# lars-frogner/Impact

Measured on AMD Instinct MI355X. Metric: voxels stepped/sec + remesh tris/sec, 512^3 grid, 1/2/4/8 MI355X, higher is better.
Workload: dtype i8 voxels, f32 SDF/mesh arithmetic, f64 moments; 1 GPU; config-2 SDF asteroid x2.05 -> 502^3 grid = 512^3 stored voxels (32768 chunks); parallelism=single GPU, voxels_per_gpu=134217728, regions=1, triangles=1813104

## Files before the change

### impact_amd/csrc/derive.hip

```cpp
#include "device_common.hpp"
#include "chunk_passes.hpp"
#include "table_roles.hpp"
#include "many.hpp"

#ifndef IVX_POL_SWEEP_PLANES
#define IVX_POL_SWEEP_PLANES IVX_ST_WT
#endif
#ifndef IVX_DERIVE_WAVES
#define IVX_DERIVE_WAVES 6
#endif

namespace {

struct DeriveParams {
    uint32_t cx, cy, cz;
};

__device__ __forceinline__ uint32_t row_mask(uint4 s) {
    uint32_t w[4] = {s.x, s.y, s.z, s.w};
    uint32_t m = 0;
#pragma unroll
    for (int q = 0; q < 4; ++q) m |= ((((w[q] >> 7) & 0x01010101u) * 0x00204081u >> 21) & 0xFu) << (4 * q);
    return m;
}

__device__ __forceinline__ uint32_t nbr_row_mask(const GridView& g, const ivx_chunk_info* info, size_t c, uint32_t off) {
    const uint32_t gen = info[c].gen_kind;
    const uint32_t rm = row_mask(*reinterpret_cast<const uint4*>(g.sdf + c * IVX_CHUNK_VOXELS + off));
    return gen == KIND_NONUNIFORM ? rm : (gen == KIND_UNIFORM ? 0xFFFFu : 0u);
}

struct ChunkPreArgs {
    GridView g;
    ivx_chunk_info* info;
    uint32_t* bbox;
    uint32_t* mesh_counts;
    uint8_t* chunk_class;
    uint8_t* touch;
    uint32_t* rparent;
    uint32_t* work_counts;
    uint32_t* next_work_count;
    uint32_t* active_list;
    ivx_roles::PresetArgs preset;
    uint32_t defer_ghost, pad_;
    unsigned long long* tick;
};
__device__ __forceinline__ void chunk_settle(const GridView& g, const ChunkPreArgs& a, uint32_t chunk, const ivx_chunk_info& own) {
    const uint32_t gen = own.gen_kind;
    const bool solid = gen == KIND_UNIFORM;
    ivx_chunk_info rec = own;
    rec.kind = (uint8_t)gen;
    rec.flags = 0;
    rec.face_dist = solid ? 0x555 : 0;
    rec.uniform_type = solid ? (own.kind == KIND_NONUNIFORM ? g.type[(size_t)chunk * IVX_CHUNK_VOXELS] : own.uniform_type) : (uint8_t)0;
    rec.region_count = solid ? 1 : 0;
    rec.boundary_region_count = solid ? 1 : 0;
    a.info[chunk] = rec;
    a.bbox[chunk] = solid ? (0x80000000u | (15u << 4) | (15u << 12) | (15u << 20)) : 0u;
    a.mesh_counts[2 * chunk] = 0;
    a.mesh_counts[2 * chunk + 1] = 0;
    a.touch[chunk] = solid ? 7 : 0;
    if (solid) a.rparent[(size_t)chunk * 256] = chunk * 256u;
}
__device__ __forceinline__ void chunk_pre_body(const ChunkPreArgs& a, uint32_t bid, uint32_t) {
    const GridView& g = a.g;
    ivx_chunk_info* __restrict__ info = a.info;
    uint32_t* __restrict__ bbox = a.bbox;
    uint32_t* __restrict__ mesh_counts = a.mesh_counts;
    uint8_t* __restrict__ chunk_class = a.chunk_class;
    uint8_t* __restrict__ touch = a.touch;
    uint32_t* __restrict__ rparent = a.rparent;
    uint32_t* __restrict__ work_counts = a.work_counts;
    uint32_t* __restrict__ next_work_count = a.next_work_count;
    uint32_t* __restrict__ active_list = a.active_list;
    __shared__ uint32_t s_w[4];
    __shared__ uint32_t s_base;
    const uint32_t tid = threadIdx.x, lane = tid & 63u, wave = tid >> 6;
    ivx_roles::role_preset(a.preset, bid * 256u + tid);
    if (bid == 0 && tid == 0) next_work_count[0] = 0u;
    const uint32_t n_chunks = g.cx * g.cy * g.cz;
    const uint32_t chunk = bid * 256u + tid;
    const bool live = chunk < n_chunks;
    bool settled = false, pending = false;
    if (live) {
        const ivx_chunk_info own = info[chunk];
        const uint32_t gen = own.gen_kind;
        settled = gen == KIND_VOID;
        if (gen == KIND_UNIFORM) {
            const int ck = chunk % g.cz, cj = (chunk / g.cz) % g.cy, ci = chunk / (g.cz * g.cy);
            if (cj > 0 && ck > 0 && cj + 1 < (int)g.cy && ck + 1 < (int)g.cz) {
                const uint32_t sx = g.cy * g.cz, sy = g.cz;
                const bool ghost_lo = ci == 0 && g.ghost_info[0] != nullptr, ghost_hi = ci + 1 == (int)g.cx && g.ghost_info[1] != nullptr;
                const bool defer = a.defer_ghost != 0u && (ghost_lo || ghost_hi);
                const bool x_lo = ci > 0 ? info[chunk - sx].gen_kind == KIND_UNIFORM : (ghost_lo && (defer || g.ghost_info[0][cj * g.cz + ck].gen_kind == KIND_UNIFORM));
                const bool x_hi =
                    ci + 1 < (int)g.cx ? info[chunk + sx].gen_kind == KIND_UNIFORM : (ghost_hi && (defer || g.ghost_info[1][cj * g.cz + ck].gen_kind == KIND_UNIFORM));
                settled = x_lo && x_hi && info[chunk - sy].gen_kind == KIND_UNIFORM && info[chunk + sy].gen_kind == KIND_UNIFORM &&
                          info[chunk - 1].gen_kind == KIND_UNIFORM && info[chunk + 1].gen_kind == KIND_UNIFORM;
                if (settled && defer) settled = false, pending = true;
            }
        }
        if (settled) chunk_settle(g, a, chunk, own);
        chunk_class[chunk] = pending ? 2 : (settled ? 1 : 0);
    }
    const bool active = live && !settled && !pending;
    const unsigned long long bal = __ballot(active);
    if (lane == 0) s_w[wave] = (uint32_t)__popcll(bal);
    __syncthreads();
    if (tid == 0) s_base = atomicAdd(&work_counts[0], (s_w[0] + s_w[1]) + (s_w[2] + s_w[3]));
    __syncthreads();
    if (active) {
        uint32_t off = s_base + (uint32_t)__popcll(bal & ((1ull << lane) - 1ull));
        for (uint32_t w = 0; w < wave; ++w) off += s_w[w];
        active_list[off] = chunk;
    }
}
__global__ __launch_bounds__(256) void k_chunk_pre(ChunkPreArgs a) {
    ivx_stage_stamp(a.tick);
    chunk_pre_body(a, blockIdx.x, gridDim.x);
}
IVX_MANY_TWIN(k_chunk_pre_many, ChunkPreArgs, chunk_pre_body, __launch_bounds__(256))
IVX_MANY_LAUNCHER(many_chunk_pre, k_chunk_pre_many, ChunkPreArgs, 256)

__global__ __launch_bounds__(256) void k_face_settle(ChunkPreArgs a) {
    const GridView& g = a.g;
    const uint32_t cols = g.cy * g.cz, t = blockIdx.x * 256u + threadIdx.x;
    if (t >= 2u * cols) return;
    const uint32_t side = t / cols, col = t % cols;
    if (side == 1u && g.cx == 1u) return;
    const uint32_t chunk = (side ? g.cx - 1u : 0u) * cols + col;
    if (a.chunk_class[chunk] != 2) return;
    const ivx_chunk_info own = a.info[chunk];
    bool uniform = true;
    if (chunk < cols && g.ghost_info[0]) uniform = uniform && g.ghost_info[0][col].gen_kind == KIND_UNIFORM;
    if (chunk >= (g.cx - 1u) * cols && g.ghost_info[1]) uniform = uniform && g.ghost_info[1][col].gen_kind == KIND_UNIFORM;
    if (uniform) {
        chunk_settle(g, a, chunk, own);
        a.chunk_class[chunk] = 1;
    } else {
        a.chunk_class[chunk] = 0;
        a.active_list[atomicAdd(&a.work_counts[0], 1u)] = chunk;
    }
}

struct DeriveLoads {
    uint2 own_rec;
    uint4 own_sd, own_types, nrow;
// ... 52 lines not shown
    const float* dens;
    double* chunk_moments;
};

struct DeriveBox {
    uint32_t n, derive_blocks;
    uint32_t lo[3], cc[3];
    uint32_t* out_list;
};
__device__ __forceinline__ void role_region_reset(uint32_t bid, const GridView& g, const DeriveBox& box, const ivx_chunk_info* __restrict__ info,
                                                  uint32_t* __restrict__ rparent, uint32_t* __restrict__ rscalar, uint32_t* __restrict__ multi_list) {
    const uint32_t chunk = bid * 256u + threadIdx.x;
    if (chunk >= g.cx * g.cy * g.cz) return;
    const uint32_t ck = chunk % g.cz, cj = (chunk / g.cz) % g.cy, ci = chunk / (g.cz * g.cy);
    if (ci - box.lo[0] < box.cc[0] && cj - box.lo[1] < box.cc[1] && ck - box.lo[2] < box.cc[2]) return;
    const uint32_t rc = info[chunk].region_count;
    for (uint32_t r = 0; r < rc; ++r) rparent[(size_t)chunk * 256 + r] = chunk * 256u + r;
    if (rc > 1u) multi_list[atomicAdd(&rscalar[2], 1u)] = chunk;
}

struct DeriveArgs {
    GridView g;
    int8_t* sdf_rw;
    uint8_t* type_rw;
    uint8_t* flags_out;
    ivx_chunk_info* info;
    uint32_t* bbox;
    uint8_t* touch;
    uint16_t* signs;
    uint8_t* kface_out;
    const uint32_t* work_counts;
    uint32_t* active_list;
    const uint32_t* list_in;
    DeriveFused fz;
    uint32_t signs_type, x_part;
    DeriveBox box;
    unsigned long long* tick;
};
template <bool SIGNS>
__device__ __forceinline__ void derive_body(const DeriveArgs& a_, uint32_t bid_, uint32_t nb_) {
    const GridView& g = a_.g;
    int8_t* __restrict__ sdf_rw = a_.sdf_rw;
    uint8_t* __restrict__ type_rw = a_.type_rw;
    uint8_t* __restrict__ flags_out = a_.flags_out;
    ivx_chunk_info* __restrict__ info = a_.info;
    uint32_t* __restrict__ bbox = a_.bbox;
    uint8_t* __restrict__ touch = a_.touch;
    uint16_t* __restrict__ signs = a_.signs;
    uint8_t* __restrict__ kface_out = a_.kface_out;
    const uint32_t* __restrict__ work_counts = a_.work_counts;
    uint32_t* __restrict__ active_list = a_.active_list;
    const uint32_t* __restrict__ list_in = a_.list_in;
    const DeriveFused& fz = a_.fz;
    const uint32_t signs_type = a_.signs_type;
    const DeriveBox& box = a_.box;
    __shared__ uint32_t occ[18][18];
    __shared__ uint32_t cnt[13];
    __shared__ CclShared s_ccl;
    __shared__ float s_dens[256];
    __shared__ uint16_t s_mtab[256];
    double (*s_red)[10] = reinterpret_cast<double (*)[10]>(s_ccl.par);
    const uint32_t tid = threadIdx.x;
    if (!SIGNS && box.n && bid_ >= box.derive_blocks) {
        role_region_reset(bid_ - box.derive_blocks, g, box, info, fz.rparent, fz.rscalar, fz.multi_list);
        return;
    }
// ... 346 lines not shown
        o[3] = r3;
        o[4] = r2 + r5;
        o[5] = r0 * cx + r5;
        o[6] = r0 * cx + r2;
        o[7] = r1 * qx;
        o[8] = r4;
        o[9] = r3 * qx;
    }
}

__device__ __forceinline__ void derive_wave_body(const DeriveArgs& a_) {
    const GridView& g = a_.g;
    uint8_t* __restrict__ flags_out = a_.flags_out;
    int8_t* __restrict__ sdf_rw = a_.sdf_rw;
    uint8_t* __restrict__ type_rw = a_.type_rw;
    ivx_chunk_info* __restrict__ info = a_.info;
    uint16_t* __restrict__ signs = a_.signs;
    uint8_t* __restrict__ kface_out = a_.kface_out;
    uint32_t* __restrict__ active_list = a_.active_list;
    const uint32_t* __restrict__ list_in = a_.list_in;
    const DeriveFused& fz = a_.fz;
    __shared__ float s_dens[256];
    __shared__ uint16_t s_mtab[256];
    __shared__ uint16_t s_occ[4][18 * 18 + 4];
    __shared__ double s_red_all[4][16][10];
    const uint32_t tid = threadIdx.x, lane = tid & 63u;
    const uint32_t wave = (uint32_t)__builtin_amdgcn_readfirstlane((int)(tid >> 6));
    uint16_t* occ = s_occ[wave];
    double (*s_red)[10] = s_red_all[wave];
    if (fz.parts & IVX_PART_MOMENTS) s_dens[tid] = fz.dens[tid], s_mtab[tid] = moments_table_entry(tid);
    __syncthreads();
    const uint32_t la = lane >> 4, j = lane & 15u;
    const uint32_t n_active = a_.work_counts[0];
    const uint32_t n_walk = gridDim.x * 4u;
    const uint32_t sx = g.cy * g.cz;
    const uint32_t* sw = reinterpret_cast<const uint32_t*>(g.signs);
    for (uint32_t li = ivx_xcd_remap(blockIdx.x, gridDim.x) * 4u + wave; li < n_active; li += n_walk) {
    IVX_TW(g, li, 0);
    const uint32_t chunk = IVX_LIST_CHUNK(list_in[li]);
    const int ck = chunk % g.cz, cj = (chunk / g.cz) % g.cy, ci = chunk / sx;
    const size_t base = (size_t)chunk * IVX_CHUNK_VOXELS;
    const bool has_zlo = ck > 0, has_zhi = ck + 1 < (int)g.cz;
    const size_t c_lo = has_zlo ? (size_t)chunk - 1 : (size_t)chunk, c_hi = has_zhi ? (size_t)chunk + 1 : (size_t)chunk;
    const uint32_t nf = la, nr = j;
    bool n_present;
    size_t nc;
    uint32_t noff;
    if (nf == 0) n_present = ci > 0, nc = (size_t)chunk - sx, noff = 240u + nr;
    else if (nf == 1) n_present = ci + 1 < (int)g.cx, nc = (size_t)chunk + sx, noff = nr;
    else if (nf == 2) n_present = cj > 0, nc = (size_t)chunk - g.cz, noff = nr * 16u + 15u;
    else n_present = cj + 1 < (int)g.cy, nc = (size_t)chunk + g.cz, noff = nr * 16u;
    if (!n_present) nc = chunk;
    uint2 own_rec = reinterpret_cast<const uint2*>(info)[chunk];
    uint32_t gen_lo = reinterpret_cast<const uint32_t*>(info)[2 * c_lo], gen_hi = reinterpret_cast<const uint32_t*>(info)[2 * c_hi];
    uint32_t ngen = reinterpret_cast<const uint32_t*>(info)[2 * nc];
    uint32_t type0 = *reinterpret_cast<const uint32_t*>(g.type + base);
    uint32_t nrow = sw[(nc * 256 + noff) >> 1];
    uint32_t ow[4], bl[4], bh[4];
#pragma unroll
    for (int q = 0; q < 4; ++q) {
        const uint32_t r = (4u * la + q) * 16u + j;
        ow[q] = sw[((size_t)chunk * 256 + r) >> 1];
        bl[q] = sw[(c_lo * 256 + r) >> 1];
        bh[q] = sw[(c_hi * 256 + r) >> 1];
    }
    asm volatile("" : "+v"(own_rec.x), "+v"(own_rec.y), "+v"(gen_lo), "+v"(gen_hi), "+v"(ngen), "+v"(type0), "+v"(nrow));
    asm volatile("" : "+v"(ow[0]), "+v"(ow[1]), "+v"(ow[2]), "+v"(ow[3]), "+v"(bl[0]), "+v"(bl[1]), "+v"(bl[2]), "+v"(bl[3]));
    asm volatile("" : "+v"(bh[0]), "+v"(bh[1]), "+v"(bh[2]), "+v"(bh[3]));
    own_rec.x = (uint32_t)__builtin_amdgcn_readfirstlane((int)own_rec.x), own_rec.y = (uint32_t)__builtin_amdgcn_readfirstlane((int)own_rec.y);
    gen_lo = ((uint32_t)__builtin_amdgcn_readfirstlane((int)gen_lo) >> 8) & 0xFFu, gen_hi = ((uint32_t)__builtin_amdgcn_readfirstlane((int)gen_hi) >> 8) & 0xFFu;
// ... 258 lines not shown
        } else {
            ci_.flags = 0;
            ci_.face_dist = 0;
        }
        info[chunk] = ci_;
    }
    IVX_TW(g, li, 5);
    ivx_wave_lds_sync();
    }
}
__global__ __launch_bounds__(256) __attribute__((amdgpu_waves_per_eu(IVX_DERIVE_WAVE_WAVES, 8))) void k_derive_wave(DeriveArgs a) {
    ivx_stage_stamp(a.tick);
    derive_wave_body(a);
}

struct ListRebuildArgs {
    GridView g;
    const ivx_chunk_info* info;
    uint32_t* work_counts;
    uint32_t* next_work_count;
    uint32_t* active_list;
    uint32_t* mesh_counts;
};
__device__ __forceinline__ void list_rebuild_body(const ListRebuildArgs& a, uint32_t bid, uint32_t) {
    const GridView& g = a.g;
    const ivx_chunk_info* __restrict__ info = a.info;
    uint32_t* __restrict__ work_counts = a.work_counts;
    uint32_t* __restrict__ next_work_count = a.next_work_count;
    uint32_t* __restrict__ active_list = a.active_list;
    uint32_t* __restrict__ mesh_counts = a.mesh_counts;
    __shared__ uint32_t s_w[4];
    __shared__ uint32_t s_base;
    const uint32_t tid = threadIdx.x, lane = tid & 63u, wave = tid >> 6;
    if (bid == 0 && tid == 0) next_work_count[0] = 0u;
    const uint32_t n_chunks = g.cx * g.cy * g.cz;
    const uint32_t chunk = bid * 256u + tid;
    const bool live = chunk < n_chunks;
    bool settled = false;
    uint32_t entry = 0;
    if (live) {
        const ivx_chunk_info own = info[chunk];
        const uint32_t gen = own.gen_kind;
        settled = gen == KIND_VOID;
        if (gen == KIND_UNIFORM) {
            const int ck = chunk % g.cz, cj = (chunk / g.cz) % g.cy, ci = chunk / (g.cz * g.cy);
            if (cj > 0 && ck > 0 && cj + 1 < (int)g.cy && ck + 1 < (int)g.cz) {
                const uint32_t sx = g.cy * g.cz, sy = g.cz;
                const bool x_lo = ci > 0 ? info[chunk - sx].gen_kind == KIND_UNIFORM
                                         : (g.ghost_info[0] != nullptr && g.ghost_info[0][cj * g.cz + ck].gen_kind == KIND_UNIFORM);
                const bool x_hi = ci + 1 < (int)g.cx ? info[chunk + sx].gen_kind == KIND_UNIFORM
                                                     : (g.ghost_info[1] != nullptr && g.ghost_info[1][cj * g.cz + ck].gen_kind == KIND_UNIFORM);
                settled = x_lo && x_hi && info[chunk - sy].gen_kind == KIND_UNIFORM && info[chunk + sy].gen_kind == KIND_UNIFORM &&
                          info[chunk - 1].gen_kind == KIND_UNIFORM && info[chunk + 1].gen_kind == KIND_UNIFORM;
            }
        }
        const uint32_t kind = own.kind;
        const bool exposed = kind == KIND_NONUNIFORM && (own.flags & CF_FULLY_OBSCURED) != CF_FULLY_OBSCURED;
        entry = chunk | (kind << 24) | (gen << 26) | (exposed ? (1u << 28) : 0u);
        if (settled) {
            mesh_counts[2 * chunk] = 0;
            mesh_counts[2 * chunk + 1] = 0;
        }
    }
    const bool active = live && !settled;
    const unsigned long long bal = __ballot(active);
    if (lane == 0) s_w[wave] = (uint32_t)__popcll(bal);
    __syncthreads();
// ... 47 lines not shown
                if (q < 6) atomicMin(&red[q], v[q]);
                else atomicMax(&red[q], v[q]);
            }
        }
        __syncthreads();
        if (tid < 6) atomicMin(&raw[tid], red[tid]);
        else if (tid < 12) atomicMax(&raw[tid], red[tid]);
    }
}

__global__ __launch_bounds__(256) void k_step_preset(ivx_roles::PresetArgs preset) { ivx_roles::role_preset(preset, blockIdx.x * 256u + threadIdx.x); }

__global__ __launch_bounds__(256) void k_materialize(uint32_t n_chunks, const ivx_chunk_info* __restrict__ info, int8_t* __restrict__ sdf,
                                                     uint8_t* __restrict__ type, uint8_t* __restrict__ flags, uint8_t* __restrict__ labels) {
    const uint32_t chunk = ivx_xcd_remap(blockIdx.x, n_chunks);
    const ivx_chunk_info ci = info[chunk];
    if (ci.kind == KIND_NONUNIFORM) return;
    const size_t o = (size_t)chunk * IVX_CHUNK_VOXELS + (size_t)threadIdx.x * 16;
    const uint32_t s = ivx_uniform_sdf(ci.kind) * 0x01010101u, t = ivx_uniform_type(ci) * 0x01010101u;
    const uint32_t f = ivx_uniform_flags(ci.kind) * 0x01010101u, l = ivx_uniform_label(ci.kind) * 0x01010101u;
    *reinterpret_cast<uint4*>(sdf + o) = make_uint4(s, s, s, s);
    *reinterpret_cast<uint4*>(type + o) = make_uint4(t, t, t, t);
    *reinterpret_cast<uint4*>(flags + o) = make_uint4(f, f, f, f);
    *reinterpret_cast<uint4*>(labels + o) = make_uint4(l, l, l, l);
}

static DeriveArgs derive_args(ivx_grid* g, const GridView& v, const DeriveFused& fz) {
    DeriveArgs da;
    memset(&da, 0, sizeof(da));
    da.g = v, da.sdf_rw = g->sdf, da.type_rw = g->type, da.flags_out = g->flags, da.info = g->info, da.bbox = g->chunk_bbox, da.touch = g->chunk_touch;
    da.signs = g->chunk_signs, da.kface_out = g->kface, da.work_counts = ivx_wc(g), da.active_list = g->active_list, da.list_in = g->active_list, da.fz = fz;
    return da;
}
static_assert(sizeof(DeriveArgs) % 8 == 0 && sizeof(ChunkPreArgs) % 8 == 0 && sizeof(ListRebuildArgs) % 8 == 0, "argument blocks travel as 8-byte words");
static const int s_many_registered_derive =
    (ivx_many_register(IVX_MK_DERIVE_PLANES, many_derive_planes, sizeof(DeriveArgs)), ivx_many_register(IVX_MK_DERIVE_SIGNS, many_derive_signs, sizeof(DeriveArgs)),
     ivx_many_register(IVX_MK_CHUNK_PRE, many_chunk_pre, sizeof(ChunkPreArgs)), ivx_many_register(IVX_MK_LIST_REBUILD, many_list_rebuild, sizeof(ListRebuildArgs)), 0);

}

int ivx_ensure_dense(ivx_grid* g) {
    if (!g->planes_compact) return IVX_OK;
    IVX_KLAUNCH(k_materialize, dim3(g->n_chunks), dim3(256), 0, g->ctx->stream, g->n_chunks, g->info, g->sdf, g->type, g->flags, g->llabel);
    IVX_HIP_CHECK(hipGetLastError());
    g->planes_compact = 0;
    return IVX_OK;
}

ivx_roles::PresetArgs ivx_preset_args(ivx_grid* g, uint32_t groups) {
    const uint32_t n_groups = (g->n_chunks + 255u) / 256u;
    ivx_roles::PresetArgs a;
    a.groups = groups;
    a.rscalar = g->rscalar;
    a.sn_sums = g->group_sums + n_groups;
    a.n_sn = IVX_SN_GROUP_WORDS * n_groups;
    a.eval_count = g->samp_len ? g->samp_len + g->n_chunks : nullptr;
    return a;
}

int ivx_launch_step_preset(ivx_grid* g, uint32_t groups) {
    if (!groups) return IVX_OK;
    const ivx_roles::PresetArgs a = ivx_preset_args(g, groups);
    IVX_KLAUNCH(k_step_preset, dim3((a.n_sn + 255u) / 256u), dim3(256), 0, g->ctx->stream, a);
    IVX_HIP_CHECK(hipGetLastError());
    g->scratch_dirty &= ~groups;
    return IVX_OK;
}

#ifdef IVX_DERIVE_DEBUG
static void derive_debug_mask() {
    static bool done = false;
    if (done) return;
    done = true;
    const char* e = getenv("IVX_DERIVE_SKIP");
    const uint32_t v = e ? (uint32_t)strtoul(e, nullptr, 0) : 0u;
    (void)hipMemcpyToSymbol(HIP_SYMBOL(ivx_dbg_derive_skip), &v, sizeof(v));
}
#endif
int ivx_launch_derive(ivx_grid* g, uint32_t parts, uint32_t preset_groups) {
#ifdef IVX_DERIVE_DEBUG
    derive_debug_mask();
#endif
    GridView v = ivx_view(g);
    DeriveFused fz;
    fz.parts = parts;
    fz.x_off = g->x_off;
    fz.labels = g->llabel;
    fz.rparent = g->rparent;
    fz.rscalar = g->rscalar;
    fz.multi_list = g->ccl_scratch;
    fz.dens = g->dens_dev;
    fz.chunk_moments = g->chunk_moments;
    if ((parts & IVX_PART_REGIONS) && !(preset_groups & IVX_SCRATCH_REGIONS) && (g->scratch_dirty & IVX_SCRATCH_REGIONS))
        IVX_HIP_CHECK(ivx_memset_async(g->rscalar, 0, 16 * sizeof(uint32_t), g->ctx->stream));
    if (parts & IVX_PART_REGIONS) g->scratch_dirty |= IVX_SCRATCH_REGIONS;
    g->bbox_valid = 1;
    uint32_t* next_count = ivx_wc(g);
    g->wc_cur ^= 1u;
    const uint32_t roll = ((g->scratch_dirty & IVX_SCRATCH_EVAL) && g->samp_len) ? IVX_SCRATCH_EVAL_ROLL : 0u;
    ChunkPreArgs face_settle;
    {
        ChunkPreArgs pa;
        memset(&pa, 0, sizeof(pa));
        pa.g = v, pa.info = g->info, pa.bbox = g->chunk_bbox, pa.mesh_counts = g->chunk_counts, pa.chunk_class = g->chunk_class, pa.touch = g->chunk_touch;
        pa.rparent = g->rparent, pa.work_counts = ivx_wc(g), pa.next_work_count = next_count, pa.active_list = g->active_list;
        pa.preset = ivx_preset_args(g, preset_groups | roll);
        if (g->ghost_event && g->ghost_split && ivx_has_interior_planes(g)) pa.defer_ghost = 1u;
        const uint32_t blocks = (g->n_chunks + 255u) / 256u;
        pa.tick = g->timing.take(ivx_many_recording());
        if (!ivx_many_try(g->ctx, g, IVX_MK_CHUNK_PRE, blocks, pa)) IVX_KLAUNCH(k_chunk_pre, dim3(blocks), dim3(256), 0, g->ctx->stream, pa);
        face_settle = pa;
        face_settle.tick = nullptr;
    }
    g->scratch_dirty &= ~preset_groups;
    if (roll) g->scratch_dirty &= ~IVX_SCRATCH_EVAL;
    uint32_t derive_grid = ivx_list_grid(g);
    if (g->last_active) {
        const uint32_t per_round = (uint32_t)g->ctx->n_cu * 32u;
        const uint32_t each = (g->last_active + per_round / 2u) / per_round > 1u ? (g->last_active + per_round / 2u) / per_round : 1u;
        derive_grid = (g->last_active + each - 1u) / each;
        const uint32_t lo = (g->n_chunks + 255u) / 256u;
        if (derive_grid < lo) derive_grid = lo;
    }
    DeriveArgs da = derive_args(g, v, fz);
    if (g->signs_current) da.signs_type = (uint32_t)g->signs_type;
    uint32_t wave_grid;
    {
        const uint32_t per_round = (uint32_t)g->ctx->n_cu * 4u * IVX_DERIVE_WAVE_WAVES;
        const uint32_t n = g->last_active ? g->last_active : per_round;
        const uint32_t each = (n + per_round / 2u) / per_round > 1u ? (n + per_round / 2u) / per_round : 1u;
        wave_grid = ((n + each - 1u) / each + 3u) / 4u;
    }
    auto sweep = [&](uint32_t x_part) {
        da.x_part = x_part;
        da.tick = g->timing.take(ivx_many_recording());
        if (g->signs_current) {
            if (ivx_many_try(g->ctx, g, IVX_MK_DERIVE_SIGNS, derive_grid, da)) return;
            if (x_part == IVX_XPART_ALL && v.ghost_sdf[0] == nullptr && v.ghost_sdf[1] == nullptr)
                IVX_KLAUNCH(k_derive_wave, dim3(wave_grid), dim3(256), 0, g->ctx->stream, da);
            else
                IVX_KLAUNCH(k_derive<true>, dim3(derive_grid), dim3(256), 0, g->ctx->stream, da);
        } else {
            if (!ivx_many_try(g->ctx, g, IVX_MK_DERIVE_PLANES, derive_grid, da)) IVX_KLAUNCH(k_derive<false>, dim3(derive_grid), dim3(256), 0, g->ctx->stream, da);
        }
    };
    if (g->ghost_event) {
        const bool interior = g->ghost_split && ivx_has_interior_planes(g);
        if (interior) sweep(IVX_XPART_INTERIOR);
        (void)ivx_many_break();
        static const bool skip_wait = getenv("IVX_DEBUG_SKIP_GHOST_WAIT") && atoi(getenv("IVX_DEBUG_SKIP_GHOST_WAIT")) == 1;
        if (!skip_wait) IVX_HIP_CHECK(hipStreamWaitEvent(g->ctx->stream, static_cast<hipEvent_t>(g->ghost_event), 0));
        g->ghost_event = nullptr;
        if (face_settle.defer_ghost) IVX_KLAUNCH(k_face_settle, dim3((2u * g->cc[1] * g->cc[2] + 255u) / 256u), dim3(256), 0, g->ctx->stream, face_settle);
        sweep(interior ? IVX_XPART_FACES : IVX_XPART_ALL);
    } else {
        sweep(IVX_XPART_ALL);
    }
    g->active_list_stale = 0;
    g->planes_compact = 1;
    IVX_HIP_CHECK(hipGetLastError());
    return IVX_OK;
}

int ivx_launch_derive_box(ivx_grid* g, uint32_t parts, const uint32_t lo[3], const uint32_t cc[3], uint32_t* d_out_list) {
    GridView v = ivx_view(g);
    DeriveFused fz;
    fz.parts = parts;
    fz.x_off = g->x_off;
    fz.labels = g->llabel;
    fz.rparent = g->rparent;
    fz.rscalar = g->rscalar;
    fz.multi_list = g->ccl_scratch;
    fz.dens = g->dens_dev;
    fz.chunk_moments = g->chunk_moments;
// ... 56 lines not shown
```

### impact_amd/csrc/ivx_api.hip

```cpp
#include <algorithm>
#include <array>
#include <functional>
#include <cmath>
#include <chrono>
#include <cstring>
#include <new>
#include <type_traits>
#include <vector>

#include "ivx_host.hpp"

static thread_local char g_error[512] = "";

void ivx_set_error(const char* fmt, ...) {
    va_list ap;
    va_start(ap, fmt);
    vsnprintf(g_error, sizeof(g_error), fmt, ap);
    va_end(ap);
}

namespace {

int ensure_host_scratch(ivx_grid* g, size_t bytes) {
    if (g->host_scratch_bytes >= bytes) return IVX_OK;
// ... 100 lines not shown
    return IVX_OK;
}

int ivx_reference_occupied(ivx_grid* g, const char* who, uint32_t occ[12]) {
    IVX_REQUIRE(g->occ_ref_valid || g->bbox_valid, IVX_ERR_STATE, "%s: the object holds no occupied ranges yet (call ivx_derive_state or a step first)", who);
    return reference_occupied(g, occ);
}

extern "C" {

const char* ivx_last_error(void) { return g_error; }

int ivx_init(int device_id, void* stream, ivx_ctx** out) {
    IVX_REQUIRE(out, IVX_ERR_INVALID, "ivx_init: null output pointer");
    *out = nullptr;
    int count = 0;
    hipError_t e = hipGetDeviceCount(&count);
    if (e != hipSuccess || count == 0) {
        ivx_set_error("ivx_init: no HIP device available (%s); this library has no CPU fallback", e == hipSuccess ? "0 devices" : hipGetErrorString(e));
        return IVX_ERR_HIP;
    }
    IVX_REQUIRE(device_id >= 0 && device_id < count, IVX_ERR_INVALID, "ivx_init: device %d out of range (0..%d)", device_id, count - 1);
    IVX_HIP_CHECK(hipSetDevice(device_id));
    hipDeviceProp_t prop;
    IVX_HIP_CHECK(hipGetDeviceProperties(&prop, device_id));
    if (strncmp(prop.gcnArchName, "gfx950", 6) != 0) {
        ivx_set_error("ivx_init: device %d is %s; this library is built for gfx950 (MI355X) only", device_id, prop.gcnArchName);
        return IVX_ERR_HIP;
    }
    ivx_ctx* c = new (std::nothrow) ivx_ctx();
    IVX_REQUIRE(c, IVX_ERR_CAPACITY, "ivx_init: out of host memory");
    c->device = device_id;
    c->n_cu = prop.multiProcessorCount > 0 ? prop.multiProcessorCount : 256;
    {
        int khz = 0;
        const hipError_t ce = hipDeviceGetAttribute(&khz, hipDeviceAttributeWallClockRate, device_id);
        if (ce != hipSuccess || khz <= 0) {
            ivx_set_error("ivx_init: the wall clock rate of device %d could not be queried (%s); stage times from clock stamps assume 100 MHz", device_id,
                          ce == hipSuccess ? "0 kHz reported" : hipGetErrorString(ce));
            khz = 100000;
        }
        c->wall_clock_khz = (double)khz;
    }
    if (stream) {
        c->stream = static_cast<hipStream_t>(stream);
        c->own_stream = false;
    } else {
        hipError_t se = hipStreamCreateWithFlags(&c->stream, hipStreamNonBlocking);
        if (se != hipSuccess) {
            ivx_set_error("ivx_init: hipStreamCreate failed: %s", hipGetErrorString(se));
            delete c;
            return IVX_ERR_HIP;
        }
        c->own_stream = true;
    }
    *out = c;
    return IVX_OK;
}

void ivx_shutdown(ivx_ctx* c) {
    if (!c) return;
    (void)ivx_stream_sync(c->stream);
    ivx_many_release(c);
    ivx_mapped_free(&c->pinned_scratch);
    ivx_buf_free(&c->dev_scratch);
    ivx_buf_free(&c->drag_scratch);
// ... 20 lines not shown
    const size_t cols = (size_t)g->cc[1] * g->cc[2];
    auto carve = [&](auto** p, size_t count) {
        using T = std::remove_pointer_t<std::remove_pointer_t<decltype(p)>>;
        const size_t bytes = (count * sizeof(T) + 255) & ~(size_t)255;
        if (arena) *p = reinterpret_cast<T*>(arena + arena_bytes);
        arena_bytes += bytes;
    };
    carve(&g->sdf, g->n_vox);
    carve(&g->type, g->n_vox);
    carve(&g->flags, g->n_vox);
    carve(&g->llabel, g->n_vox);
    carve(&g->info, (size_t)g->n_chunks);
    carve(&g->chunk_bbox, (size_t)g->n_chunks);
    for (int sd = 0; sd < 2; ++sd) {
        carve(&g->ghost_sdf[sd], cols * 256);
        carve(&g->ghost_type[sd], cols * 256);
        carve(&g->ghost_info[sd], cols);
    }
    carve(&g->chunk_counts, (size_t)g->n_chunks * 2);
    carve(&g->chunk_offsets, (size_t)g->n_chunks * 3 + 8);
    carve(&g->partials, g->partial_blocks * 10 + 16);
    carve(&g->rparent, (size_t)g->n_chunks * 256);
    carve(&g->rcompid, (size_t)g->n_chunks * 256);
    carve(&g->rscalar, (size_t)64);
    carve(&g->ccl_scratch, (size_t)g->n_chunks * 2);
    carve(&g->sn_list, (size_t)g->n_chunks * 4);
    carve(&g->group_sums, (size_t)((g->n_chunks + 255u) / 256u) * (1u + IVX_SN_GROUP_WORDS) + IVX_SN_TAIL_WORDS);
    carve(&g->sn_hard, (size_t)g->n_chunks);
    carve(&g->sn_walk, (size_t)g->n_chunks * 5 + 2);
    carve(&g->dens_dev, (size_t)256);
    carve(&g->work_counts, (size_t)8);
    carve(&g->occ_part, (size_t)((g->n_chunks + 255u) / 256u) * 12 + 12);
    carve(&g->active_list, (size_t)g->n_chunks);
    carve(&g->chunk_class, (size_t)g->n_chunks);
    carve(&g->chunk_touch, (size_t)g->n_chunks);
    carve(&g->chunk_signs, (size_t)g->n_chunks * 256);
    carve(&g->kface, (size_t)g->n_chunks * 1024);
    carve(&g->chunk_moments, (size_t)g->n_chunks * 10);
    return arena_bytes;
}
static int grid_new(ivx_ctx* c, const uint32_t cc[3], float voxel_extent, uint32_t x_chunk_offset, uint32_t global_x_chunks, ivx_grid** out) {
    IVX_REQUIRE(c && cc && out, IVX_ERR_INVALID, "ivx_grid_create: null argument");
    *out = nullptr;
    IVX_REQUIRE(cc[0] > 0 && cc[1] > 0 && cc[2] > 0, IVX_ERR_INVALID, "ivx_grid_create: empty chunk grid");
    IVX_REQUIRE(voxel_extent > 0.0f, IVX_ERR_INVALID, "ivx_grid_create: voxel extent must be positive");
    const uint64_t n64 = (uint64_t)cc[0] * cc[1] * cc[2];
    IVX_REQUIRE(n64 <= (1u << 24), IVX_ERR_CAPACITY, "ivx_grid_create: more than 2^24 chunks");
    ivx_grid* g = new (std::nothrow) ivx_grid();
    IVX_REQUIRE(g, IVX_ERR_CAPACITY, "ivx_grid_create: out of host memory");
    memset(g, 0, sizeof(*g));
    g->scratch_dirty = IVX_SCRATCH_REGIONS;
    g->ctx = c;
    for (int d = 0; d < 3; ++d) g->cc[d] = cc[d];
    g->n_chunks = (uint32_t)n64;
    g->n_vox = (size_t)n64 * IVX_CHUNK_VOXELS;
    g->extent = voxel_extent;
    g->x_off = x_chunk_offset;
    g->gx = global_x_chunks ? global_x_chunks : cc[0];
    g->partial_blocks = 2048;
    *out = g;
    return IVX_OK;
}

int ivx_grid_create(ivx_ctx* c, const uint32_t cc[3], float voxel_extent, uint32_t x_chunk_offset, uint32_t global_x_chunks, ivx_grid** out) {
    ivx_grid* g = nullptr;
    int rc = grid_new(c, cc, voxel_extent, x_chunk_offset, global_x_chunks, &g);
// ... 127 lines not shown
    IVX_REQUIRE(g && out, IVX_ERR_INVALID, "ivx_grid_chunk_counts: null argument");
    for (int d = 0; d < 3; ++d) out[d] = g->cc[d];
    return IVX_OK;
}

int ivx_grid_stage_counters(ivx_grid* g, uint32_t out[4]) {
    IVX_REQUIRE(g && out, IVX_ERR_INVALID, "ivx_grid_stage_counters: null argument");
    for (int i = 0; i < 4; ++i) out[i] = 0;
    int rc;
    if (g->samp_len) {
        uint32_t ev[3];
        if ((rc = d2h(g, ev, g->samp_len + g->n_chunks + ((g->scratch_dirty & IVX_SCRATCH_EVAL) ? 0 : 8), sizeof(ev)))) return rc;
        out[0] = ev[0] + ev[1] + ev[2];
    }
    if ((rc = d2h(g, &out[1], g->rscalar + 2, sizeof(uint32_t)))) return rc;
    if ((rc = d2h(g, &out[2], g->chunk_offsets + 2 * (size_t)g->n_chunks + 2, sizeof(uint32_t)))) return rc;
    out[3] = g->n_chunks;
    return IVX_OK;
}

void* ivx_grid_device_ptr(ivx_grid* g, int which) {
    if (!g) return nullptr;
    if (which >= 0 && which < 4 && ivx_ensure_dense(g) != IVX_OK) return nullptr;
    if (which == 0 || which == 1 || which == 4) ivx_planes_touched(g);
    switch (which) {
        case 0: return g->sdf;
        case 1: return g->type;
        case 2: return g->flags;
        case 3: return g->llabel;
        case 4: return g->info;
        case 5: return g->rparent;
#ifdef IVX_WG_TRACE
        case 6: return g->chunk_moments;
#endif
        case 7: return g->samp_len;
        case 8: return g->samp_ops;
        case 10: return g->sn_hard;
        case 9: return ivx_sn_hard_count(g);
        default: return nullptr;
    }
}

int ivx_sdf_sample(ivx_grid* g, const ivx_sdf_processed_node* nodes, size_t n_nodes, uint32_t stack_size, const uint32_t grid_shape[3],
                   const float shifted_grid_center[3], uint8_t voxel_type) {
    IVX_REQUIRE(g && grid_shape && shifted_grid_center, IVX_ERR_INVALID, "ivx_sdf_sample: null argument");
    IVX_REQUIRE(n_nodes == 0 || nodes, IVX_ERR_INVALID, "ivx_sdf_sample: null node array");
    for (int d = 0; d < 3; ++d) {
        const uint32_t cap = (d == 0 ? g->gx : g->cc[d]) * 16u;
        IVX_REQUIRE(grid_shape[d] <= cap, IVX_ERR_INVALID, "ivx_sdf_sample: grid shape %u exceeds the chunk grid (%u voxels) along axis %d", grid_shape[d], cap, d);
    }
    int depth = 0, max_depth = 0;
    for (size_t i = 0; i < n_nodes; ++i) {
        const uint32_t k = nodes[i].kind;
        IVX_REQUIRE(k <= 9, IVX_ERR_INVALID, "ivx_sdf_sample: unsupported node kind %u", k);
        IVX_REQUIRE(k != 6 || nodes[i].reserved[1] <= 255u, IVX_ERR_INVALID, "ivx_sdf_sample: noise node with more than 255 octaves");
        if (k <= 2) max_depth = std::max(max_depth, ++depth);
        else if (k >= 7) {
            IVX_REQUIRE(depth >= 2, IVX_ERR_INVALID, "ivx_sdf_sample: malformed node program (combination without two operands)");
            --depth;
        } else if (k == 5 || k == 6) {
            IVX_REQUIRE(depth >= 1, IVX_ERR_INVALID, "ivx_sdf_sample: malformed node program (scaling / noise without operand)");
        }
    }
    IVX_REQUIRE(n_nodes == 0 || depth == 1, IVX_ERR_INVALID, "ivx_sdf_sample: malformed node program (final stack depth %d)", depth);
    IVX_REQUIRE((uint32_t)max_depth <= stack_size || n_nodes == 0, IVX_ERR_INVALID, "ivx_sdf_sample: stack_size %u < required %d", stack_size, max_depth);
    int rc;
// ... 675 lines not shown
```

### impact_amd/csrc/ivx_internal.hpp

```cpp
#pragma once
#include <hip/hip_runtime.h>

#include <cstdarg>
#include <cstdint>
#include <cstdio>
#include <cstring>

#include "../../include/impact_voxel_hip.h"
#include "many.hpp"
#include "stage_clock.hpp"

static inline hipError_t ivx_memset_async(void* p, int v, size_t n, hipStream_t s) {
    (void)ivx_many_break();
    return hipMemsetAsync(p, v, n, s);
}
static inline hipError_t ivx_memcpy_async(void* d, const void* src, size_t n, hipMemcpyKind k, hipStream_t s) {
    (void)ivx_many_break();
    return hipMemcpyAsync(d, src, n, k, s);
}
static inline hipError_t ivx_stream_sync(hipStream_t s) {
    (void)ivx_many_break();
    return hipStreamSynchronize(s);
}
static inline hipError_t ivx_memcpy_sync(void* d, const void* src, size_t n, hipMemcpyKind k) {
// ... 13 lines not shown
#define VF_X_DN 0x04u
#define VF_Y_DN 0x08u
#define VF_Z_DN 0x10u
#define VF_X_UP 0x20u
#define VF_Y_UP 0x40u
#define VF_Z_UP 0x80u
#define CF_ONLY_EMPTY 0x40u
#define CF_FULLY_OBSCURED 0x3Fu
#define KIND_VOID 0
#define KIND_UNIFORM 1
#define KIND_NONUNIFORM 2
#define FD_EMPTY 0
#define FD_FULL 1
#define FD_MIXED 2
#define TYPE_DUMMY 255
#define SD_VOID_LIMIT 100

struct ivx_buf {
    void* p = nullptr;
    size_t bytes = 0;
};
struct ivx_mapped {
    void* p = nullptr;
    void* dev = nullptr;
    size_t bytes = 0;
};

struct ivx_ctx {
    int device;
    hipStream_t stream;
    bool own_stream;
    int n_cu;
    double wall_clock_khz;
    ivx_mapped pinned_scratch;
    ivx_buf dev_scratch;
    hipStream_t aux_stream;
    void* many_recorder;
    int many_error;
    ivx_buf drag_scratch;
    void* cull_state;
    void* bvol_state;
};

struct ivx_block {
    void* dev;
    void* pinned;
    int refs;
};

struct ivx_grid {
    ivx_ctx* ctx;
    uint32_t cc[3];
    uint32_t n_chunks;
    size_t n_vox;
    float extent;
    uint32_t x_off, gx;
    char* arena;
    ivx_block* arena_block;
    ivx_block* host_block;
    int8_t* sdf;
    uint8_t* type;
    uint8_t* flags;
    uint8_t* llabel;
    ivx_chunk_info* info;
    uint32_t* chunk_bbox;
    int8_t* ghost_sdf[2];
// ... 2 lines not shown
    int has_ghost[2];
    void* ghost_event;
    int ghost_split;
    void* face_ids_event;
    const uint8_t* ghost_ext[2];
    uint32_t* chunk_counts;
    uint32_t* chunk_offsets;
    float* positions;
    float* normals;
    uint32_t* indices;
    uint8_t* index_materials;
    uint8_t* vertex_materials;
    ivx_submesh* submeshes;
    size_t vcap, icap, scap;
    ivx_mesh_counts mesh_counts;
    int mesh_valid;
    double* partials;
    size_t partial_blocks;
    uint32_t* rparent;
    uint32_t* rcompid;
    uint32_t* rscalar;
    uint32_t* ccl_scratch;
    uint32_t* sn_list;
    uint32_t* group_sums;
    uint32_t* sn_walk;
    uint32_t* sn_hard;
    uint32_t region_count;
    int regions_valid;
    uint32_t* work_counts;
    uint32_t wc_cur;
    uint32_t scratch_dirty;
    uint32_t* occ_part;
    uint32_t* active_list;
    uint8_t* chunk_class;
    uint8_t* kface;
    uint16_t* chunk_signs;
    uint8_t* chunk_touch;
    double* chunk_moments;
    uint32_t last_active;
    int planes_compact;
    int signs_current;
    uint8_t signs_type;
    int active_list_stale;
    int regions_labelled_locally;
    struct ivx_edit_state* edit;
    uint32_t post1_needs_box[12];
    const uint32_t* post1_needs_touched;
    uint32_t* post1_needs_out;
    int early_needs_on;
    uint32_t* post1_needs_early;
    uint32_t* post1_needs_counter;
    uint32_t* post1_needs_bell;
    uint32_t post1_needs_seq;
    const uint32_t* gather_copy_src;
    uint32_t* gather_copy_dst;
    uint32_t gather_copy_words;
    uint64_t gather_flush_id;
    int gather_launched;
    int sn_tail_zero;
    int needs_current;
    float* dens_call;
    float* dens_dev;
    float dens_host[256];
    void* dev_scratch;
    size_t dev_scratch_bytes;
    ivx_sdf_processed_node* prog_nodes;
// ... 348 lines not shown
```

Baseline: 891.9 billion voxels/s.

## Schedule costly nonuniform chunks first in derive wave sweep via order list

The chunk pre-pass now splits active chunks into costly (nonuniform) and cheap groups with two extra atomic counters. It writes an order permutation that puts costly chunks at the front and cheap ones at the back. k_derive_wave walks its work through this permutation so expensive chunks start first and cheap ones fill the tail, which should cut load imbalance at the end of the sweep. In exchange it adds an indirection load per chunk and drops the XCD remap on the ordered path, which may hurt cache locality.

```diff
diff --git a/impact_amd/csrc/derive.hip b/impact_amd/csrc/derive.hip
--- a/impact_amd/csrc/derive.hip
+++ b/impact_amd/csrc/derive.hip
@@ -1,5 +1,6 @@
 #include "device_common.hpp"
 #include "chunk_passes.hpp"
+#include "sweep_order.hpp"
 #include "table_roles.hpp"
 #include "many.hpp"
 
@@ -41,6 +42,7 @@
     uint32_t* work_counts;
     uint32_t* next_work_count;
     uint32_t* active_list;
+    uint32_t* order;
     ivx_roles::PresetArgs preset;
     uint32_t defer_ghost, pad_;
     unsigned long long* tick;
@@ -73,19 +75,21 @@
     uint32_t* __restrict__ work_counts = a.work_counts;
     uint32_t* __restrict__ next_work_count = a.next_work_count;
     uint32_t* __restrict__ active_list = a.active_list;
-    __shared__ uint32_t s_w[4];
-    __shared__ uint32_t s_base;
+    uint32_t* __restrict__ order = a.order;
+    __shared__ uint32_t s_w[4], s_wf[4];
+    __shared__ uint32_t s_base[3];
     const uint32_t tid = threadIdx.x, lane = tid & 63u, wave = tid >> 6;
     ivx_roles::role_preset(a.preset, bid * 256u + tid);
-    if (bid == 0 && tid == 0) next_work_count[0] = 0u;
+    if (bid == 0 && tid < 3u) next_work_count[2u * tid] = 0u;
     const uint32_t n_chunks = g.cx * g.cy * g.cz;
     const uint32_t chunk = bid * 256u + tid;
     const bool live = chunk < n_chunks;
-    bool settled = false, pending = false;
+    bool settled = false, pending = false, costly = false;
     if (live) {
         const ivx_chunk_info own = info[chunk];
         const uint32_t gen = own.gen_kind;
         settled = gen == KIND_VOID;
+        costly = gen == KIND_NONUNIFORM;
         if (gen == KIND_UNIFORM) {
             const int ck = chunk % g.cz, cj = (chunk / g.cz) % g.cy, ci = chunk / (g.cz * g.cy);
             if (cj > 0 && ck > 0 && cj + 1 < (int)g.cy && ck + 1 < (int)g.cz) {
@@ -104,15 +108,24 @@
         chunk_class[chunk] = pending ? 2 : (settled ? 1 : 0);
     }
     const bool active = live && !settled && !pending;
-    const unsigned long long bal = __ballot(active);
-    if (lane == 0) s_w[wave] = (uint32_t)__popcll(bal);
+    const unsigned long long bal = __ballot(active), balf = __ballot(active && costly);
+    if (lane == 0) s_w[wave] = (uint32_t)__popcll(bal), s_wf[wave] = (uint32_t)__popcll(balf);
     __syncthreads();
-    if (tid == 0) s_base = atomicAdd(&work_counts[0], (s_w[0] + s_w[1]) + (s_w[2] + s_w[3]));
+    if (tid < (order ? 3u : 1u)) {
+        const uint32_t all = (s_w[0] + s_w[1]) + (s_w[2] + s_w[3]), front = (s_wf[0] + s_wf[1]) + (s_wf[2] + s_wf[3]);
+        s_base[tid] = atomicAdd(&work_counts[2u * tid], tid == 0u ? all : (tid == 1u ? front : all - front));
+    }
     __syncthreads();
     if (active) {
-        uint32_t off = s_base + (uint32_t)__popcll(bal & ((1ull << lane) - 1ull));
+        const unsigned long long below = (1ull << lane) - 1ull;
+        uint32_t off = s_base[0] + (uint32_t)__popcll(bal & below);
         for (uint32_t w = 0; w < wave; ++w) off += s_w[w];
         active_list[off] = chunk;
+        if (order) {
+            uint32_t place = s_base[costly ? 1 : 2] + (uint32_t)__popcll((costly ? balf : bal & ~balf) & below);
+            for (uint32_t w = 0; w < wave; ++w) place += costly ? s_wf[w] : s_w[w] - s_wf[w];
+            order[costly ? place : n_chunks - 1u - place] = off;
+        }
     }
 }
 __global__ __launch_bounds__(256) void k_chunk_pre(ChunkPreArgs a) {
@@ -231,6 +244,7 @@
     const uint32_t* work_counts;
     uint32_t* active_list;
     const uint32_t* list_in;
+    const uint32_t* order;
     DeriveFused fz;
     uint32_t signs_type, x_part;
     DeriveBox box;
@@ -643,10 +657,13 @@
     __syncthreads();
     const uint32_t la = lane >> 4, j = lane & 15u;
     const uint32_t n_active = a_.work_counts[0];
-    const uint32_t n_walk = gridDim.x * 4u;
     const uint32_t sx = g.cy * g.cz;
     const uint32_t* sw = reinterpret_cast<const uint32_t*>(g.signs);
-    for (uint32_t li = ivx_xcd_remap(blockIdx.x, gridDim.x) * 4u + wave; li < n_active; li += n_walk) {
+    const uint32_t* __restrict__ order = a_.order;
+    const uint32_t n_front = order ? a_.work_counts[IVX_WC_FRONT] : 0u, n_chunks = sx * g.cx;
+    const uint32_t n_walk = ivx_sweep_stride(gridDim.x);
+    for (uint32_t t = ivx_sweep_first(order ? blockIdx.x : ivx_xcd_remap(blockIdx.x, gridDim.x), wave); t < n_active; t += n_walk) {
+    const uint32_t li = order ? (uint32_t)__builtin_amdgcn_readfirstlane((int)order[ivx_sweep_order_index(t, n_front, n_chunks)]) : t;
     IVX_TW(g, li, 0);
     const uint32_t chunk = IVX_LIST_CHUNK(list_in[li]);
     const int ck = chunk % g.cz, cj = (chunk / g.cz) % g.cy, ci = chunk / sx;
@@ -971,7 +988,7 @@
     __shared__ uint32_t s_w[4];
     __shared__ uint32_t s_base;
     const uint32_t tid = threadIdx.x, lane = tid & 63u, wave = tid >> 6;
-    if (bid == 0 && tid == 0) next_work_count[0] = 0u;
+    if (bid == 0 && tid < 3u) next_work_count[2u * tid] = 0u;
     const uint32_t n_chunks = g.cx * g.cy * g.cz;
     const uint32_t chunk = bid * 256u + tid;
     const bool live = chunk < n_chunks;
@@ -1085,6 +1102,7 @@
     da.signs = g->chunk_signs, da.kface_out = g->kface, da.work_counts = ivx_wc(g), da.active_list = g->active_list, da.list_in = g->active_list, da.fz = fz;
     return da;
 }
+static_assert(IVX_WC_FRONT == 2u && IVX_WC_BACK == 4u, "k_chunk_pre and k_list_rebuild address the three counters as words 2 t");
 static_assert(sizeof(DeriveArgs) % 8 == 0 && sizeof(ChunkPreArgs) % 8 == 0 && sizeof(ListRebuildArgs) % 8 == 0, "argument blocks travel as 8-byte words");
 static const int s_many_registered_derive =
     (ivx_many_register(IVX_MK_DERIVE_PLANES, many_derive_planes, sizeof(DeriveArgs)), ivx_many_register(IVX_MK_DERIVE_SIGNS, many_derive_signs, sizeof(DeriveArgs)),
@@ -1151,12 +1169,14 @@
     uint32_t* next_count = ivx_wc(g);
     g->wc_cur ^= 1u;
     const uint32_t roll = ((g->scratch_dirty & IVX_SCRATCH_EVAL) && g->samp_len) ? IVX_SCRATCH_EVAL_ROLL : 0u;
+    const bool ordered = g->signs_current && !g->ghost_event && v.ghost_sdf[0] == nullptr && v.ghost_sdf[1] == nullptr && !ivx_many_recording() && !g->ctx->sweep_order_off;
     ChunkPreArgs face_settle;
     {
         ChunkPreArgs pa;
         memset(&pa, 0, sizeof(pa));
         pa.g = v, pa.info = g->info, pa.bbox = g->chunk_bbox, pa.mesh_counts = g->chunk_counts, pa.chunk_class = g->chunk_class, pa.touch = g->chunk_touch;
         pa.rparent = g->rparent, pa.work_counts = ivx_wc(g), pa.next_work_count = next_count, pa.active_list = g->active_list;
+        pa.order = ordered ? g->sweep_order : nullptr;
         pa.preset = ivx_preset_args(g, preset_groups | roll);
         if (g->ghost_event && g->ghost_split && ivx_has_interior_planes(g)) pa.defer_ghost = 1u;
         const uint32_t blocks = (g->n_chunks + 255u) / 256u;
@@ -1189,10 +1209,12 @@
         da.tick = g->timing.take(ivx_many_recording());
         if (g->signs_current) {
             if (ivx_many_try(g->ctx, g, IVX_MK_DERIVE_SIGNS, derive_grid, da)) return;
-            if (x_part == IVX_XPART_ALL && v.ghost_sdf[0] == nullptr && v.ghost_sdf[1] == nullptr)
+            if (x_part == IVX_XPART_ALL && v.ghost_sdf[0] == nullptr && v.ghost_sdf[1] == nullptr) {
+                da.order = ordered ? g->sweep_order : nullptr;
                 IVX_KLAUNCH(k_derive_wave, dim3(wave_grid), dim3(256), 0, g->ctx->stream, da);
-            else
+            } else {
                 IVX_KLAUNCH(k_derive<true>, dim3(derive_grid), dim3(256), 0, g->ctx->stream, da);
+            }
         } else {
             if (!ivx_many_try(g->ctx, g, IVX_MK_DERIVE_PLANES, derive_grid, da)) IVX_KLAUNCH(k_derive<false>, dim3(derive_grid), dim3(256), 0, g->ctx->stream, da);
         }
diff --git a/impact_amd/csrc/ivx_api.hip b/impact_amd/csrc/ivx_api.hip
--- a/impact_amd/csrc/ivx_api.hip
+++ b/impact_amd/csrc/ivx_api.hip
@@ -156,6 +156,7 @@
     IVX_REQUIRE(c, IVX_ERR_CAPACITY, "ivx_init: out of host memory");
     c->device = device_id;
     c->n_cu = prop.multiProcessorCount > 0 ? prop.multiProcessorCount : 256;
+    c->sweep_order_off = getenv("IVX_DEBUG_NO_SWEEP_ORDER") && atoi(getenv("IVX_DEBUG_NO_SWEEP_ORDER")) == 1;
     {
         int khz = 0;
         const hipError_t ce = hipDeviceGetAttribute(&khz, hipDeviceAttributeWallClockRate, device_id);
@@ -242,6 +243,7 @@
     carve(&g->work_counts, (size_t)8);
     carve(&g->occ_part, (size_t)((g->n_chunks + 255u) / 256u) * 12 + 12);
     carve(&g->active_list, (size_t)g->n_chunks);
+    carve(&g->sweep_order, (size_t)g->n_chunks);
     carve(&g->chunk_class, (size_t)g->n_chunks);
     carve(&g->chunk_touch, (size_t)g->n_chunks);
     carve(&g->chunk_signs, (size_t)g->n_chunks * 256);
@@ -435,6 +437,7 @@
         case 5: return g->rparent;
 #ifdef IVX_WG_TRACE
         case 6: return g->chunk_moments;
+        case 11: return g->active_list;
 #endif
         case 7: return g->samp_len;
         case 8: return g->samp_ops;
diff --git a/impact_amd/csrc/ivx_internal.hpp b/impact_amd/csrc/ivx_internal.hpp
--- a/impact_amd/csrc/ivx_internal.hpp
+++ b/impact_amd/csrc/ivx_internal.hpp
@@ -69,6 +69,7 @@
     bool own_stream;
     int n_cu;
     double wall_clock_khz;
+    bool sweep_order_off;
     ivx_mapped pinned_scratch;
     ivx_buf dev_scratch;
     hipStream_t aux_stream;
@@ -137,6 +138,7 @@
     uint32_t scratch_dirty;
     uint32_t* occ_part;
     uint32_t* active_list;
+    uint32_t* sweep_order;
     uint8_t* chunk_class;
     uint8_t* kface;
     uint16_t* chunk_signs;
diff --git a/impact_amd/csrc/sweep_order.hpp b/impact_amd/csrc/sweep_order.hpp
--- /dev/null
+++ b/impact_amd/csrc/sweep_order.hpp
@@ -0,0 +1,16 @@
+#pragma once
+#include <stdint.h>
+
+#if defined(__HIPCC__) || defined(__HIP__)
+#define IVX_SWEEP_FN __host__ __device__ __forceinline__
+#else
+#define IVX_SWEEP_FN inline
+#endif
+
+#define IVX_WC_FRONT 2u
+#define IVX_WC_BACK 4u
+
+IVX_SWEEP_FN uint32_t ivx_sweep_first(uint32_t b, uint32_t wave) { return b * 4u + wave; }
+IVX_SWEEP_FN uint32_t ivx_sweep_stride(uint32_t nb) { return nb * 4u; }
+
+IVX_SWEEP_FN uint32_t ivx_sweep_order_index(uint32_t t, uint32_t n_front, uint32_t n_chunks) { return t < n_front ? t : n_chunks - 1u - (t - n_front); }
```

Measured after the change: 903.7 billion voxels/s, median of 4. About the same (+1.3%).
